# gsanya/orbslam2_NMI

Hardware: AMD Instinct MI355X
Metric: pose-candidate NMI evals/sec (640x480, 256 bins), one blocking nmi_search_grid call per step incl. its 8-byte read-back (SURVEY.md 8d's definition); beside the W warm-up steps an untimed clock warm-up of clock_warmup_ms = 200 ms precedes the timed region (higher is better)
Workload: dtype u8

## Files before the change

### orbslam2_nmi_amd/csrc/nmi_capi.cpp

```cpp
#include <sched.h>

#include "nmi_ctx.h"

namespace nmi_internal {

int hip_fail(nmi_ctx *ctx, hipError_t e, const char *what)
{
    if (ctx) {
        char buf[256];
        snprintf(buf, sizeof buf, "%s: %s (%d)", what, hipGetErrorString(e), (int)e);
        ctx->detail = buf;
    }
    return NMI_ERR_HIP - (int)e;
}



void build_order(int S, int Wn, int *order)
{
    const int tile_s = S >= 8 ? 8 : (S >= 4 ? 4 : (S >= 2 ? 2 : 1)), tile_w = 32 / tile_s;
    int64_t o = 0;
    for (int w0 = 0; w0 < Wn; w0 += tile_w)
        for (int s0 = 0; s0 < S; s0 += tile_s)
            for (int w = w0; w < w0 + tile_w && w < Wn; ++w)
                for (int s = s0; s < s0 + tile_s && s < S; ++s) order[o++] = w * S + s;
}

int ensure_order(nmi_ctx *ctx, int S, int Wn, const int **d_order)
{
    *d_order = nullptr;
    if (!ctx->xcd_tiling) return NMI_OK;
    const int64_t total = (int64_t)S * Wn;
    nmi_ctx::OrderEntry *victim = nullptr;
    for (auto &e : ctx->orders) {
        if (e.S == S && e.Wn == Wn) {
            e.last_use = ++ctx->order_clock;
            *d_order = e.d.as<int>();
            return NMI_OK;
        }
        if (!victim || (!e.d && victim->d) || (!e.d == !victim->d && e.last_use < victim->last_use)) victim = &e;
    }
    nmi_ctx::OrderEntry &e = *victim;
    if (e.d) NMI_HIP_TRY(ctx, hipStreamSynchronize(ctx->stream));
    e.S = e.Wn = -1;
    const size_t bytes = (size_t)total * sizeof(int);
    NMI_HIP_TRY(ctx, e.d.grow(bytes));
    NMI_HIP_TRY(ctx, e.h.grow(bytes, nmi_mem::kPinned));
    build_order(S, Wn, e.h.as<int>());
    NMI_HIP_TRY(ctx, hipMemcpyAsync(e.d.as<int>(), e.h.as<int>(), bytes, hipMemcpyHostToDevice, ctx->stream));
    e.S = S;
    e.Wn = Wn;
    e.last_use = ++ctx->order_clock;
    *d_order = e.d.as<int>();
    return NMI_OK;
}

nmi::PlanInputs plan_inputs(const nmi_ctx *ctx, nmi::SearchForm form, int64_t total, const nmi::GridArgs &a)
{
    nmi::PlanInputs in;
    in.compute_units = ctx->compute_units;
    in.workgroups = ctx->workgroups;
    in.hist_variant = ctx->hist_variant;
    in.split_mode = ctx->split_mode;
    in.split_pixels = ctx->split_pixels;
    in.shift = ctx->shift;
    in.use_bg = ctx->params.use_bg != 0;
    in.phase_mask = ctx->phase_mask;
    in.content_path = ctx->content_path;
    in.xcd_tiling = ctx->xcd_tiling != 0;
    in.cooldown = ctx->split_cooldown > 0;
    in.few_hint = ctx->few_hint;
    in.total = total;
    in.width = a.width;
    in.npix = ctx->npix;
    in.vec_ok = a.vec_ok != 0;
    in.form = form;
    return in;
}

double pix_owner_share(const nmi_ctx *ctx, int pix)
{
    const double owner_px = ((double)ctx->npix + (double)(pix - 1) * ctx->pix_owner_bias) / pix;
    return owner_px < ctx->npix ? owner_px / ctx->npix : 1.0;
}

static int ensure_pix_timeouts(nmi_ctx *ctx)
{
    NMI_HIP_TRY(ctx, ctx->d_pix_timeouts.grow(nmi::kPixHealWords * sizeof(uint32_t), ctx->stream, true));
    return NMI_OK;
}

static int next_split_epoch(nmi_ctx *ctx, uint32_t *epoch)
{
    uint32_t e = ctx->split_epoch + 1;
    if ((e & 0xFFFFu) == 0) {
        if (ctx->d_blocks) NMI_HIP_TRY(ctx, hipMemsetAsync(ctx->d_blocks.as<>(), 0, ctx->d_blocks.size(), ctx->stream));
        if (ctx->d_pix_blocks) NMI_HIP_TRY(ctx, hipMemsetAsync(ctx->d_pix_blocks.as<>(), 0, ctx->d_pix_blocks.size(), ctx->stream));
        if (e == 0 && ctx->d_slabs) NMI_HIP_TRY(ctx, hipMemsetAsync(ctx->d_slabs.as<>(), 0, ctx->d_slabs.size(), ctx->stream));
        ++e;
    }
    ctx->split_epoch = *epoch = e;
    return NMI_OK;
}

int prepare_pix_handoff(nmi_ctx *ctx, uint32_t *epoch)
{
    if (*epoch == 0) {
        const int rc = next_split_epoch(ctx, epoch);
        if (rc != NMI_OK) return rc;
    }
    return ensure_pix_timeouts(ctx);
}

static int ensure_zeroed(nmi_ctx *ctx, DeviceBuffer &buf, size_t bytes)
{
    NMI_HIP_TRY(ctx, buf.grow(bytes, ctx->stream, true));
    return NMI_OK;
}

int prepare_search(nmi_ctx *ctx, const nmi::SearchPlan &plan, nmi::GridArgs &a)
{
    const int64_t total = (int64_t)a.S_local * a.Wn;
    int rc = NMI_OK;
    if (plan.kind == nmi::SearchKernel::split) {
        rc = ensure_zeroed(ctx, ctx->d_slabs, (size_t)(total > 128 ? total : 128) * sizeof(nmi::SplitSlab));
        if (rc == NMI_OK && plan.pix_parts > 1) rc = ensure_zeroed(ctx, ctx->d_blocks, (size_t)total * nmi::split_block_bytes_per_candidate(plan.pix_parts));
        if (rc == NMI_OK) rc = next_split_epoch(ctx, &a.epoch);
        a.slabs = ctx->d_slabs.as<nmi::SplitSlab>();
        a.blocks = ctx->d_blocks.as<unsigned long long>();
        a.split_error = ctx->split_error.device<uint32_t>();
    } else if (plan.kind == nmi::SearchKernel::pix) {
        rc = ensure_zeroed(ctx, ctx->d_pix_blocks, nmi::pix_block_bytes((int)total, plan.pix));
        if (rc == NMI_OK) rc = prepare_pix_handoff(ctx, &a.epoch);
        a.blocks = ctx->d_pix_blocks.as<unsigned long long>();
    } else if (plan.order_table) {
        rc = ensure_order(ctx, a.S_local, a.Wn, &a.order);
    }
    if (rc != NMI_OK) return rc;
#ifdef NMI_BUILD_ABLATIONS
    if (plan.scratch && plan.workgroups > ctx->scratch_workgroups) {
        ctx->scratch_workgroups = 0;
        const int alloc = plan.workgroups > ctx->compute_units ? plan.workgroups : ctx->compute_units;
        NMI_HIP_TRY(ctx, ctx->d_scratch.grow(nmi::grid_kernel_scratch_bytes(alloc), ctx->stream));
        ctx->scratch_workgroups = alloc;
        a.scratch = ctx->d_scratch.as<uint32_t>();
    }
#endif
    if (plan.probe) a.plan = ctx->d_plan.as<nmi::LevelPlan>();
    if (plan.kind == nmi::SearchKernel::few_levels) {
        const size_t need = (size_t)(a.S_local + a.Wn) * (size_t)ctx->npix;
        if (need > ctx->d_rank_stacks.size()) NMI_HIP_TRY(ctx, ctx->d_rank_stacks.grow(need + need / 2, ctx->stream));
    }
    return NMI_OK;
}

int commit_launch(nmi_ctx *ctx, bool post, bool post_score, const SearchLaunch &rec, bool launched, SearchLaunch *out)
{
    if (post) ++ctx->seq;
    if (post_score) ++ctx->pair_seq;
    ctx->posted = post;
    ctx->last_slot = ctx->slot;
    ctx->last = rec;
    if (out) *out = rec;
    if (!launched) return NMI_OK;
    ctx->slot ^= 1;
    if (ctx->profiling) {
        NMI_HIP_TRY(ctx, hipEventRecord(ctx->ev_stop, ctx->stream));
        ctx->have_timing = true;
    }
    return NMI_OK;
}

nmi::GridArgs grid_args(const nmi_ctx *ctx, const SearchRequest &rq, bool post, bool post_score)
{
    const nmi_params &p = ctx->params;
    nmi::GridArgs a{};
    a.render_stack = rq.render_stack;
    a.warp_stack = rq.warp_stack;
    a.S_local = rq.S_local;
    a.Wn = rq.Wn;
    a.s_offset = rq.s_offset;
    a.S_total = rq.S_total;
    a.w_offset = rq.w_offset;
    nmi::set_geometry(a, p.width, p.height, rq.render_stack, rq.warp_stack, p.render_bottom_up != 0);
    a.shift = ctx->shift;
    a.mode = p.mode;
    a.ratings = rq.d_ratings;
    a.key = ctx->d_keys.as<unsigned long long>() + ctx->slot;
    a.reset_key = ctx->d_keys.as<unsigned long long>() + (ctx->slot ^ 1);
    a.out_key = rq.out_key;
    a.done = ctx->d_done.as<unsigned int>();
    a.mailbox = post ? ctx->mailbox.as<nmi::Mailbox>() : nullptr;
    a.score_post = post_score ? ctx->score_mailbox.as<unsigned long long>() : nullptr;
    a.seq = post ? ctx->seq + 1 : (post_score ? ctx->pair_seq + 1 : 0);
    a.hist_variant = ctx->hist_variant;
    return a;
}

int enqueue_grid(nmi_ctx *ctx, const SearchRequest &rq, SearchLaunch *launched)
{
    const nmi_params &p = ctx->params;
    const bool post = rq.post && ctx->result_path == 1, post_score = rq.post_score && ctx->result_path == 1;
    nmi::GridArgs a = grid_args(ctx, rq, post, post_score);
    if (rq.pair_renders) {
        a.pair_renders = rq.pair_renders;
        a.pair_warps = rq.pair_warps;
        uintptr_t bits = 0;
        for (int i = 0; i < rq.S_local; ++i) bits |= (uintptr_t)rq.pair_renders_host[i] | (uintptr_t)rq.pair_warps_host[i];
        if (bits % 16) nmi::set_geometry(a, p.width, p.height, (const void *)1, (const void *)1, p.render_bottom_up != 0);
    }
    a.table = ctx->table.as<float>();
    a.scratch = ctx->d_scratch.as<uint32_t>();
    a.dbg_joint = rq.dbg_joint;
    a.dbg_h1 = rq.dbg_h1;
    a.dbg_h2 = rq.dbg_h2;
    a.dbg_sums = rq.dbg_sums;
    a.dbg_stamps = ctx->dbg_stamps;

    const int64_t total = (int64_t)rq.S_local * rq.Wn;
// ... 673 lines not shown
```

### orbslam2_nmi_amd/csrc/nmi_ctx.h

```cpp
#pragma once
#include <hip/hip_runtime.h>
#include <math.h>
#include <stdio.h>
#include <string.h>

#include <new>
#include <string>
#include <vector>

#include "nmi_hip.h"
#include "nmi_covered.h"
#include "nmi_kernels.h"
#include "nmi_masked.h"
#include "nmi_mem.h"
#include "nmi_search_plan.h"
#include "nmi_tone.h"

struct SearchLaunch {
    nmi::SearchKernel kind = nmi::SearchKernel::none;
    int parts = 0;
    int pix = 0;
    uint32_t epoch = 0;
    int few = 0;
};

using nmi_mem::DeviceBuffer;
using nmi_mem::PinnedBuffer;

struct MeshWorkArea {
    DeviceBuffer zbuf, bins, state, clip_queue, clip_state, pairs, pair_state;
    nmi::MeshWork view;
};

struct nmi_ctx {
    nmi_params params{};
    int device = 0;
    int compute_units = 0;
    int npix = 0;
    int shift = 0;
    nmi_mem::Stream own_stream;
    hipStream_t stream = nullptr;
    DeviceBuffer table;
    DeviceBuffer d_keys;
    PinnedBuffer h_key;
    DeviceBuffer d_done;
    PinnedBuffer mailbox;
    unsigned int seq = 0;
    int slot = 0;
    int last_slot = 0;
    SearchLaunch last;
    int pix_owner_bias = 49152;
    DeviceBuffer d_pix_timeouts;
    uint32_t split_timeouts = 0;
    uint32_t split_cooldown = 0;
    uint32_t split_backoff = kSplitBackoffMin;
    uint32_t split_cooldown_epoch = 0;
    static constexpr uint32_t kSplitBackoffMin = 16, kSplitBackoffMax = 4096;
    int result_path = 1;
    bool posted = false;
    DeviceBuffer d_pair_rating;
    DeviceBuffer d_reduced_key;
    PinnedBuffer score_mailbox;
    unsigned int pair_seq = 0;
    int wait_mode = 0;
    struct OrderEntry {
        int S = -1, Wn = -1;
        DeviceBuffer d;
        PinnedBuffer h;
        uint64_t last_use = 0;
    };
    static constexpr int kOrderCache = 16;
    OrderEntry orders[kOrderCache];
    uint64_t order_clock = 0;
    int xcd_tiling = 1;
    DeviceBuffer d_slabs;
    DeviceBuffer d_blocks;
    uint32_t split_epoch = 0;
    PinnedBuffer split_error;
    DeviceBuffer d_pix_blocks;
    PinnedBuffer pair_table;
    DeviceBuffer d_pair_scores;
    int pairs_cap = 0;
    int split_pixels = -1;
    DeviceBuffer d_plan;
    PinnedBuffer level_post;
    uint32_t level_seq = 0;
    uint32_t level_seen = 0;
    bool few_hint = false;
    int content_path = -1;
    int fewlevels_bins = 4096;
    DeviceBuffer d_rank_stacks;
    unsigned long long *dbg_stamps = nullptr;
    int stamp_candidate = 0;
    int split_mode = -1;
    DeviceBuffer d_zbuf;
    DeviceBuffer d_no_red;
    MeshWorkArea mesh;
    int mesh_views = 0;
    unsigned long long tile_queue_limit = 4ull << 20;
    unsigned long long clip_queue_limit = ~0ull;
    nmi_mem::UploadRing mvp_ring, warp_ring;
    DeviceBuffer d_scratch;
    int scratch_workgroups = 0;
    DeviceBuffer d_mask_counts;
    DeviceBuffer d_mask_tables;
    int mask_count_n = 0;
    DeviceBuffer d_mask_redo;
    DeviceBuffer d_mask_redo_state;
    DeviceBuffer d_cover_counts;
    int64_t cover_count_n = 0;
    nmi::ToneSetting tone;
    nmi_internal::ToneWork tone_work;
    nmi::ValidRange valid;
    nmi_mem::Event ev_start, ev_stop;
    int hist_variant = 3;
    int phase_mask = 3;
    int workgroups = 0;
    bool profiling = false;
    bool have_timing = false;
    std::string detail;
};

struct nmi_texture {
    nmi_ctx *ctx = nullptr;
    DeviceBuffer d_luma;
    int levels = 0;
    int w[16] = {}, h[16] = {};
    long long off[16] = {};
};

namespace nmi_internal {

int mesh_work_alloc(nmi_ctx *ctx, int S, MeshWorkArea *w);
int ensure_mesh_work(nmi_ctx *ctx, int S);
int ensure_mesh_pairs(nmi_ctx *ctx, MeshWorkArea *w, long long n_triangles);
int warp_inverse_coeffs(const double *forward , float *coeffs );
int point_sprite_size(float point_size, int *size);
int level_enqueue(nmi_level *lv, const float *h_mvps, const double *h_forward, const unsigned long long **d_key);
nmi_ctx *level_ctx(nmi_level *lv);
int rccl_allreduce_key(nmi_ctx *ctx, const unsigned long long *d_send, unsigned long long *d_recv, void *nccl_comm);

int hip_fail(nmi_ctx *ctx, hipError_t e, const char *what);
void build_order(int S, int Wn, int *order);
int ensure_order(nmi_ctx *ctx, int S, int Wn, const int **d_order);
struct SearchRequest {
    const uint8_t *render_stack = nullptr, *warp_stack = nullptr;
    int S_local = 0, s_offset = 0, S_total = 0, Wn = 0, w_offset = 0;
    float *d_ratings = nullptr;
    unsigned long long *out_key = nullptr;
    bool post = false;
    bool post_score = false;
    uint32_t *dbg_joint = nullptr, *dbg_h1 = nullptr, *dbg_h2 = nullptr;
    float *dbg_sums = nullptr;
    bool caller_checks_split = false;
    const uint8_t *const *pair_renders = nullptr, *const *pair_warps = nullptr;
    const uint8_t *const *pair_renders_host = nullptr, *const *pair_warps_host = nullptr;
    static SearchRequest block(const uint8_t *renders, int S_local, int s_offset, int S_total, const uint8_t *warps, int Wn, int w_offset = 0)
    {
        SearchRequest rq;
        rq.render_stack = renders;
        rq.warp_stack = warps;
        rq.S_local = S_local;
        rq.s_offset = s_offset;
        rq.S_total = S_total;
        rq.Wn = Wn;
        rq.w_offset = w_offset;
        return rq;
    }
};
struct MaskSide {
    const uint8_t *warp_masks = nullptr, *render_masks = nullptr;
    int32_t *counts = nullptr;
    const float *tables = nullptr;
    int32_t *redo = nullptr;
    uint32_t *redo_state = nullptr;
};
nmi::GridArgs grid_args(const nmi_ctx *ctx, const SearchRequest &rq, bool post, bool post_score);
nmi::PlanInputs plan_inputs(const nmi_ctx *ctx, nmi::SearchForm form, int64_t total, const nmi::GridArgs &a);
double pix_owner_share(const nmi_ctx *ctx, int pix);
int prepare_pix_handoff(nmi_ctx *ctx, uint32_t *epoch);
int prepare_search(nmi_ctx *ctx, const nmi::SearchPlan &plan, nmi::GridArgs &a);
int commit_launch(nmi_ctx *ctx, bool post, bool post_score, const SearchLaunch &rec, bool launched, SearchLaunch *out);
int enqueue_grid(nmi_ctx *ctx, const SearchRequest &rq, SearchLaunch *launched = nullptr);
struct MaskSearch {
    bool covered;
    nmi::MaskedGridArgs masked;
    nmi::CoveredGridArgs cover;
};
MaskSearch mask_search_args(const nmi::GridArgs &a, const MaskSide &m);
hipError_t launch_mask_search(const MaskSearch &ms, int pix, double owner_share, int workgroups, bool use_bg, bool exact,
                              const uint32_t *replay, uint32_t *healed, hipStream_t stream);
int ensure_mask_redo(nmi_ctx *ctx, int64_t total);
int enqueue_grid_mask(nmi_ctx *ctx, const SearchRequest &rq, const MaskSide &m, SearchLaunch *launched = nullptr);
int wait_word(nmi_ctx *ctx, const volatile unsigned long long *word, unsigned long long mask, unsigned long long want,
              unsigned long long *out);
int stage_floats(nmi_ctx *ctx, nmi_mem::UploadRing &ring, const float *h_src, size_t n, float **d_out);
int fetch_key(nmi_ctx *ctx, unsigned long long *key);
bool split_timed_out(nmi_ctx *ctx);
bool split_launch_failed(nmi_ctx *ctx, const SearchLaunch &launch);
extern const char *const kSplitTimeoutNote, *const kSplitTimeoutTicketNote, *const kSplitTimeoutTicketLost;
int search_block(nmi_ctx *ctx, const uint8_t *render_stack, int32_t S_local, int32_t s_offset, int32_t S_total, const uint8_t *warp_stack,
                 int32_t Wn_local, int32_t w_offset, int32_t Wn_total, float *d_ratings, uint64_t *d_key, uint64_t *h_key,
                 bool caller_checks);
enum class MapKind { points, textured_mesh, colored_mesh };
int render_points_impl(nmi_ctx *ctx, const float *d_xyz, const float *d_red, int64_t n_points, const float *h_mvps, int32_t S,
                       float point_size, uint8_t *d_render_stack, uint8_t *cover, const nmi::DepthShade *depth = nullptr);
int render_mesh_impl(nmi_ctx *ctx, MapKind kind, const float *d_xyz, const float *d_attr, int64_t n_triangles, const nmi_texture *tex,
                     const float *h_mvps, int32_t S, uint8_t *d_render_stack, uint8_t *cover, const nmi::DepthShade *depth = nullptr);
int depth_shade_check(const nmi_depth_shade *shade, nmi::DepthShade *out);
nmi::MeshShading mesh_shading(MapKind kind, const float *d_attr, const nmi_texture *tex);
nmi::RenderTarget render_target(const nmi_ctx *ctx, uint8_t *out, uint8_t *cover, const nmi::DepthShade *depth);
nmi::MeshLimits mesh_limits(const nmi_ctx *ctx, int layout_views);
int check_grid_args(nmi_ctx *ctx, const uint8_t *render_stack, int S_local, int s_offset, int S_total, const uint8_t *warp_stack,
                    int Wn);

#define NMI_HIP_TRY(ctx, call)                                  \
    do {                                                        \
        hipError_t e_ = (call);                                 \
        if (e_ != hipSuccess) return nmi_internal::hip_fail((ctx), e_, #call); \
    } while (0)

struct FirstError {
    hipError_t e = hipSuccess;
    bool operator()(hipError_t r)
    {
        if (e == hipSuccess) e = r;
        return r == hipSuccess;
// ... 18 lines not shown
```

### orbslam2_nmi_amd/csrc/nmi_grid_device.h

```cpp
#pragma once
#include <hip/hip_runtime.h>
#include <stdint.h>

#include "nmi_kernels.h"
#include "nmi_device.h"

namespace nmi {

namespace {

constexpr int kBlock = NMI_BLOCK_THREADS;
constexpr int kWaves = kBlock / 64;
constexpr int kBins = 256;
constexpr int kWords = kBins * kBins / 2;
constexpr int kRowStride = 129;
constexpr int kJointWords = kBins * kRowStride;
constexpr int kOvfCap = 1024;
constexpr int kRowsPerWave = kBins / kWaves;
constexpr int kLdsTable = 4096;
constexpr int kSide = 8;


struct Lds {
    uint32_t joint[kJointWords];
// ... 260 lines not shown
                const int cn = min(ch + kStep, last);
                const uint4 wn = ldw(cn), rn = ldr(cn);
                add_chunk<BG, SHIFTED, HIST, true>(lds, par, rc, wc, a.shift, try_flat);
                wc = wn;
                rc = rn;
            }
        }
        if (ROWS && row_rem > 0) {
            const int x0 = a.chunks_per_row << 4, n = a.height * row_rem;
            for (int t = tid; t < n; t += NT) {
                const int y = t / row_rem, x = x0 + t - y * row_rem;
                const int ry = a.flip ? (a.height - 1 - y) : y;
                uint32_t d1 = render[ry * a.width + x], d2 = warped[y * a.width + x];
                if (HIST == 2) {
                    if (BG || (d1 != 0 && d2 != 0)) {
                        if (SHIFTED) {
                            d1 >>= a.shift;
                            d2 >>= a.shift;
                        }
                        (void)__hip_atomic_fetch_add(&lds.joint[joint_word(d1, d2)], joint_inc(d2), __ATOMIC_RELAXED, __HIP_MEMORY_SCOPE_WORKGROUP);
                    }
                } else {
                    add_pixel<BG, SHIFTED>(lds, par, d1, d2, a.shift);
                }
            }
        }
    } else {
        for (int pos = tid; pos < a.npix; pos += NT) {
            const int y = pos / a.width;
            const int x = pos - y * a.width;
            const int ry = a.flip ? (a.height - 1 - y) : y;
            if (HIST == 2) {
                uint32_t d1 = render[ry * a.width + x], d2 = warped[pos];
                if (BG || (d1 != 0 && d2 != 0)) {
                    if (SHIFTED) {
                        d1 >>= a.shift;
                        d2 >>= a.shift;
                    }
                    (void)__hip_atomic_fetch_add(&lds.joint[joint_word(d1, d2)], joint_inc(d2), __ATOMIC_RELAXED,
                                                 __HIP_MEMORY_SCOPE_WORKGROUP);
                }
            } else {
                add_pixel<BG, SHIFTED>(lds, par, render[ry * a.width + x], warped[pos], a.shift);
            }
        }
    }
}

__device__ __forceinline__ float term(const float *__restrict__ table, uint32_t c)
{
    return c ? table[c] : 0.0f;
}
__device__ __forceinline__ float term_lds(const Lds &lds, const float *__restrict__ table, uint32_t c)
{
    float t = lds.table[c < (uint32_t)kLdsTable ? c : 0u];
    if (__builtin_expect(c >= (uint32_t)kLdsTable, 0)) t = table[c];
    return t;
}

static_assert(kWaves == 16 && (kWaves * kRowStride) % 32 == 16, "rows kWaves apart must fall on opposite halves of the 32 banks");
__device__ __forceinline__ int decode_row(int wave, int pass, int r) { return wave + 4 * kWaves * pass + kWaves * r; }
__device__ __forceinline__ bool in_decode_pass(uint32_t d1, int wave, int pass)
{
    return (d1 % (uint32_t)kWaves) == (uint32_t)wave && (d1 / (uint32_t)(4 * kWaves)) == (uint32_t)pass;
}
__device__ __forceinline__ uint32_t decode_word(int d1, int i, int k) { return (uint32_t)(d1 * kRowStride + i + 16 * k); }

__device__ __forceinline__ void apply_wraps(const Lds &lds, int par, uint32_t novf, uint32_t word, uint32_t &lo,
                                            uint32_t &hi)
{
    for (uint32_t e = 0; e < novf; ++e) {
        const uint32_t ev = lds.ovf[par][e];
        if ((ev >> 1) == word) {
            if (ev & 1u) {
                hi += 65536u;
            } else {
                lo += 65536u;
                hi -= 1u;
            }
        }
    }
}

template <bool ZERO0 = false>
__device__ __forceinline__ void decode_phase(Lds &lds, int par, const GridArgs &a, int wave, int lane)
{
    const uint32_t novf = lds.ovf_n[par] < (uint32_t)kOvfCap ? lds.ovf_n[par] : (uint32_t)kOvfCap;
    const bool side_any = lds.side_key[par][0] != 0u;
    uint32_t wave_total = 0;
    const int i = lane & 15, r = lane >> 4;
    uint32_t col_lo[8], col_hi[8];
#pragma unroll
    for (int k = 0; k < 8; ++k) col_lo[k] = col_hi[k] = 0;
#pragma unroll 1
    for (int pass = 0; pass < kRowsPerWave / 4; ++pass) {
        const int d1 = decode_row(wave, pass, r);
        const uint32_t a0 = decode_word(d1, i, 0);
        uint32_t lo[8], hi[8];
#pragma unroll
        for (int k = 0; k < 8; ++k) {
            const uint32_t idx = a0 + 16 * k;
            const uint32_t wd = lds.joint[idx];
            lds.joint[idx] = 0;
            lo[k] = wd & 0xFFFFu;
            hi[k] = wd >> 16;
        }
        if (__builtin_expect(novf != 0, 0)) {
#pragma unroll
            for (int k = 0; k < 8; ++k) apply_wraps(lds, par, novf, a0 + 16 * k, lo[k], hi[k]);
        }
        if (__builtin_expect(side_any, 0)) {
            for (int e = 0; e < kSide; ++e) {
                const uint32_t key1 = __builtin_amdgcn_readfirstlane(lds.side_key[par][e]);
                if (key1 == 0u) break;
                const uint32_t sd1 = (key1 - 1u) >> 8, sd2 = (key1 - 1u) & 0xFFu;
                if (!in_decode_pass(sd1, wave, pass)) continue;
                const uint32_t sword = joint_word(sd1, sd2);
                const uint32_t cnt = lds.side_cnt[par][e];
#pragma unroll
                for (int k = 0; k < 8; ++k) {
                    if (a0 + 16 * k == sword) {
                        if (sd2 & 128u)
                            hi[k] += cnt;
                        else
                            lo[k] += cnt;
                    }
                }
            }
        }
        uint32_t rsum = 0, cmax = 0;
        if (ZERO0) {
            uint32_t raw = 0;
#pragma unroll
            for (int k = 0; k < 8; ++k) raw += lo[k] + hi[k];
            wave_total += row_sum_16(raw);
            if (i == 0) lo[0] = 0;
            if (d1 == 0) {
#pragma unroll
                for (int k = 0; k < 8; ++k) lo[k] = hi[k] = 0;
            }
        }
        float tl[8], th[8];
#pragma unroll
        for (int k = 0; k < 8; ++k) {
            col_lo[k] += lo[k];
            col_hi[k] += hi[k];
            rsum += lo[k] + hi[k];
            cmax = max(cmax, max(lo[k], hi[k]));
            tl[k] = lds.table[lo[k] & (kLdsTable - 1)];
            th[k] = lds.table[hi[k] & (kLdsTable - 1)];
        }
        if (__builtin_expect(cmax >= (uint32_t)kLdsTable, 0)) {
#pragma unroll
            for (int k = 0; k < 8; ++k) {
                if (lo[k] >= (uint32_t)kLdsTable) tl[k] = a.table[lo[k]];
                if (hi[k] >= (uint32_t)kLdsTable) th[k] = a.table[hi[k]];
            }
        }
        rsum = row_sum_16(rsum);
        if (!ZERO0) wave_total += rsum;
        const float x = row_tree_16(lane_tree_16(tl, th));
        if (i == 0) {
            lds.hist_render[d1] = rsum;
            lds.joint_row_sums[d1] = x;
        }
        if (a.dbg_joint) {
            uint32_t *row = a.dbg_joint + d1 * kBins;
#pragma unroll
            for (int k = 0; k < 8; ++k) {
                const int q = i + 16 * k;
                row[q] = lo[k];
                row[q + 128] = hi[k];
            }
        }
    }
#pragma unroll
    for (int k = 0; k < 8; ++k) {
        const int q = i + 16 * k;
        atomicAdd(&lds.hist_warped[q], col_lo[k]);
        atomicAdd(&lds.hist_warped[q + 128], col_hi[k]);
    }
    if (i == 0) atomicAdd(&lds.total[par], wave_total);
}

__device__ __forceinline__ void final_phase(Lds &lds, const GridArgs &a, int lane, int p, int w, int s,
                                            unsigned long long &prev_key)
{
    const int i = lane & 15, r = lane >> 4;
    float lo[8], hi[8];
    const uint32_t *h = r == 0 ? lds.hist_render : lds.hist_warped;
    uint32_t cl[8], ch[8];
#pragma unroll
    for (int k = 0; k < 8; ++k) {
        cl[k] = r < 2 ? h[i + 16 * k] : 0u;
        ch[k] = r < 2 ? h[i + 16 * k + 128] : 0u;
    }
#pragma unroll
    for (int k = 0; k < 8; ++k) {
        lo[k] = a.table[cl[k]];
        hi[k] = a.table[ch[k]];
    }
    if ((w == 0 || s == 0) && a.plan) {
        uint32_t m = 0;
#pragma unroll
        for (int k = 0; k < 8; ++k) m |= (cl[k] != 0u ? 1u << k : 0u) | (ch[k] != 0u ? 0x100u << k : 0u);
        if (lane < 32 && m) __hip_atomic_fetch_or(const_cast<uint32_t *>(&a.plan->seen[lane]), m, __ATOMIC_RELAXED, __HIP_MEMORY_SCOPE_AGENT);
    }
    if (r == 2) {
#pragma unroll
        for (int k = 0; k < 8; ++k) {
            lo[k] = lds.joint_row_sums[i + 16 * k];
            hi[k] = lds.joint_row_sums[i + 16 * k + 128];
        }
    }
    const float x = row_tree_16(lane_tree_16(lo, hi));
    const float a1 = __shfl(x, 0, 64), a2 = __shfl(x, 16, 64), a3 = __shfl(x, 32, 64);
    if (a.dbg_h1 && lane < 64) {
        for (int t = lane; t < kBins; t += 64) {
            a.dbg_h1[t] = lds.hist_render[t];
            if (a.dbg_h2) a.dbg_h2[t] = lds.hist_warped[t];
        }
    }
    if (lane == 0) commit_score(a, p, w, s, a1, a2, a3, prev_key);
}

__device__ __forceinline__ void finish_search(const GridArgs &a, int lane, unsigned long long prev_key, uint32_t expected)
{
    LevelPlan *plan = const_cast<LevelPlan *>(a.plan);
    uint32_t arrived = 0;
    if (lane == 0) {
        const unsigned int one = prev_key == ~0ull ? 2u : 1u;
        arrived = __hip_atomic_fetch_add(a.done, one, __ATOMIC_RELAXED, __HIP_MEMORY_SCOPE_AGENT);
    }
    if (__builtin_amdgcn_readfirstlane(arrived) != expected - 1) return;
    unsigned long long final_key = 0;
    uint32_t bits = 0;
    unsigned long long *post = nullptr;
    uint32_t state = 0, max_joint = 0;
    if (lane == 0) final_key = __hip_atomic_load(a.key, __ATOMIC_RELAXED, __HIP_MEMORY_SCOPE_AGENT);
    if (plan && lane < 32) bits = __hip_atomic_exchange(&plan->seen[lane], 0u, __ATOMIC_RELAXED, __HIP_MEMORY_SCOPE_AGENT);
    if (plan && lane == 0) post = plan->seen_post, state = plan->seen_state, max_joint = plan->seen_max_joint;
    if (lane == 0) {
        __hip_atomic_store(a.done, 0u, __ATOMIC_RELAXED, __HIP_MEMORY_SCOPE_AGENT);
        if (a.out_key) __hip_atomic_store(a.out_key, final_key, __ATOMIC_RELAXED, __HIP_MEMORY_SCOPE_SYSTEM);
        if (a.mailbox)
            __hip_atomic_store(&a.mailbox->word, final_key | ((unsigned long long)(a.seq & 1u) << 63), __ATOMIC_RELAXED, __HIP_MEMORY_SCOPE_SYSTEM);
    }
    if (plan) {
        const uint32_t n = row_sum_16((uint32_t)__popc(bits));
        const uint32_t nw = (uint32_t)__shfl((int)n, 16, 64);
        const uint32_t few = (n > 0u && nw > 0u && n * nw <= max_joint) ? 1u : 0u;
        if (lane == 0 && post && few != state) {
            plan->seen_state = few;
            const uint32_t stamp = 0x80000000u | (uint32_t)wall_clock64();
            __hip_atomic_store(post, ((unsigned long long)stamp << 32) | ((unsigned long long)n << 16) | nw, __ATOMIC_RELAXED, __HIP_MEMORY_SCOPE_SYSTEM);
        }
    }
}

template <bool SHIFTED, bool BG = true, bool ROWS = false>
__device__ __forceinline__ void exact_candidate(Lds &lds, const GridArgs &a, int tid, int p, unsigned long long &prev_key)
{
    const int lane = tid & 63, wave = tid >> 6;
    const int w = p / a.S_local, s = p - w * a.S_local;
    __syncthreads();
    histogram_phase<true, SHIFTED, 1, kBlock, true, ROWS>(lds, 0, a, a.render_stack + (size_t)s * a.npix, a.warp_stack + (size_t)w * a.npix, tid, 0,
                                                          ROWS ? a.height * a.chunks_per_row : a.npix >> 4);
    __syncthreads();
    decode_phase<!BG>(lds, 0, a, wave, lane);
    __syncthreads();
    if (wave == 0) {
        final_phase(lds, a, lane, p, w, s, prev_key);
        for (int t = lane; t < kBins; t += 64) lds.hist_warped[t] = 0;
        if (lane == 0) lds.ovf_n[0] = lds.total[0] = 0;
        if (lane < kSide) lds.side_key[0][lane] = lds.side_cnt[0][lane] = 0;
    }
    __syncthreads();
}

}

}
```

### orbslam2_nmi_amd/csrc/nmi_kernels.hip

```cpp
#include <hip/hip_runtime.h>
#include <stdint.h>

#include "nmi_grid_device.h"

namespace nmi {

#if defined(NMI_GRID_KERNEL_GATED)
#define NMI_GRID_KERNEL_NAME nmi_grid_kernel_gated
#elif defined(NMI_GRID_KERNEL_STAMPED)
#define NMI_GRID_KERNEL_NAME nmi_grid_kernel_stamped
#elif defined(NMI_GRID_KERNEL_ROWS)
#define NMI_GRID_KERNEL_NAME nmi_grid_kernel_rows
#else
#define NMI_GRID_KERNEL_NAME nmi_grid_kernel
#endif
#ifdef NMI_GRID_KERNEL_STAMPED
#define NMI_GRID_STAMP(k)                                                                                         \
    do {                                                                                                          \
        if (a.dbg_stamps && tid == ((k) == 7 ? 64 : 0) && stamp_on) a.dbg_stamps[blockIdx.x * 8 + (k)] = wall_clock64(); \
    } while (0)
#else
#define NMI_GRID_STAMP(k) \
    do {                  \
    } while (0)
#endif
#ifndef NMI_WAVE_SLABS
#define NMI_WAVE_SLABS 1
#endif
#ifdef NMI_GRID_KERNEL_STAMPED
namespace {
__device__ uint32_t stamp_candidate = 0;
}
#endif
template <bool BG, bool SHIFTED, int HIST>
__global__ __launch_bounds__(NMI_BLOCK_THREADS) void NMI_GRID_KERNEL_NAME(GridArgs a)
{
    __shared__ Lds lds;
#ifdef NMI_GRID_KERNEL_GATED
    if (a.plan->use != 0u) return;
#endif
    const int tid = threadIdx.x;
    const int lane = tid & 63;
    const int wave = tid >> 6;
#ifdef NMI_GRID_KERNEL_STAMPED
    bool stamp_on = true;
    const int stamp_ordinal = slot_in_round(blockIdx.x, gridDim.x) + (int)stamp_candidate * (int)gridDim.x;
#endif
    NMI_GRID_STAMP(0);
    constexpr bool kOptimistic = HIST == 3;
    constexpr int kFirst = kOptimistic ? 2 : HIST;
#ifdef NMI_GRID_KERNEL_ROWS
    constexpr bool kRows = true;
#define NMI_ALL_CHUNKS (a.height * a.chunks_per_row)
#else
    constexpr bool kRows = false;
#define NMI_ALL_CHUNKS (a.npix >> 4)
#endif
    constexpr bool kZero0 = !BG && kOptimistic && !SHIFTED;
    constexpr bool kCountAll = BG || kZero0;
    constexpr bool kSlabs = NMI_WAVE_SLABS != 0 && kFirst == 2;

    if (blockIdx.x == 0 && tid == 0 && a.reset_key) *a.reset_key = 0ull;
    float tab[kLdsTable / kBlock];
#pragma unroll
    for (int k = 0; k < kLdsTable / kBlock; ++k) {
        const int c = tid + k * kBlock;
        tab[k] = a.table[c <= a.npix ? c : 0];
    }
    {
        uint4 *j4 = reinterpret_cast<uint4 *>(lds.joint);
        const uint4 z = {0, 0, 0, 0};
        for (int i = tid; i < kJointWords / 4; i += kBlock) j4[i] = z;
    }
    if (tid < kBins) lds.hist_warped[tid] = 0;
    if (tid < 2) lds.ovf_n[tid] = lds.total[tid] = 0;
    if (tid < 2 * kSide) (&lds.side_key[0][0])[tid] = (&lds.side_cnt[0][0])[tid] = 0;
    bool table_pending = true;
    int exact_from = -1;
    __syncthreads();
    NMI_GRID_STAMP(1);

    const int total = a.S_local * a.Wn;
    unsigned long long prev_key = 0;
    int par = 0;
    const int slot = slot_in_round(blockIdx.x, gridDim.x);
    int ordinal = slot;
    for (; ordinal < total; ordinal += gridDim.x, par ^= 1) {
        const int p = candidate_at(a, ordinal);
        const int w = p / a.S_local;
        const int s = p - w * a.S_local;
        const uint8_t *render = a.render_stack + (size_t)s * a.npix;
        const uint8_t *warped = a.warp_stack + (size_t)w * a.npix;
#ifdef NMI_GRID_KERNEL_STAMPED
        stamp_on = ordinal == stamp_ordinal;
#endif
        NMI_GRID_STAMP(7);

        if (a.phase_mask & 1) {
            if (a.phase_mask & 8) {
                if (wave < kWaves / 2) histogram_phase<kCountAll, SHIFTED, kFirst, kBlock / 2, true, kRows>(lds, par, a, render, warped, tid, 0, NMI_ALL_CHUNKS);
            } else
                histogram_phase<kCountAll, SHIFTED, kFirst, kBlock, true, kRows, kSlabs>(lds, par, a, render, warped, tid, 0, NMI_ALL_CHUNKS, ordinal != slot);
        }
        if (table_pending) {
#pragma unroll
            for (int k = 0; k < kLdsTable / kBlock; ++k) lds.table[tid + k * kBlock] = tab[k];
            table_pending = false;
        }
        NMI_GRID_STAMP(2);
#ifdef NMI_GRID_KERNEL_STAMPED
        if (a.dbg_stamps && lane == 0 && stamp_on) a.dbg_stamps[gridDim.x * 8 + blockIdx.x * 16 + wave] = wall_clock64();
#endif
        __syncthreads();
        NMI_GRID_STAMP(3);
        if (a.phase_mask & 2) decode_phase<kZero0>(lds, par, a, wave, lane);
        __syncthreads();
        NMI_GRID_STAMP(4);
        if (kOptimistic && (a.phase_mask & 3) == 3 && lds.total[par] != (uint32_t)a.npix) {
            exact_from = ordinal;
            break;
        }
        if (wave == 0) {
            if (a.phase_mask & 2) final_phase(lds, a, lane, p, w, s, prev_key);
            for (int t = lane; t < kBins; t += 64) lds.hist_warped[t] = 0;
            if (lane == 0) {
                lds.ovf_n[par] = 0;
                lds.total[par ^ 1] = 0;
            }
            if (lane < kSide) {
                int l = lane;
                asm volatile("" : "+v"(l));
                lds.side_key[par][l] = lds.side_cnt[par][l] = 0;
            }
        }
        NMI_GRID_STAMP(5);
    }

    if (kOptimistic && exact_from >= 0) {
        __syncthreads();
        if (tid < kBins) lds.hist_warped[tid] = 0;
        if (tid < 2) lds.total[tid] = lds.ovf_n[tid] = 0;
        if (tid < 2 * kSide) (&lds.side_key[0][0])[tid] = (&lds.side_cnt[0][0])[tid] = 0;
        __syncthreads();
        for (int o = exact_from; o < total; o += gridDim.x) exact_candidate<SHIFTED, !kZero0, kRows>(lds, a, tid, candidate_at(a, o), prev_key);
    }

    if (wave == 0 && !(a.phase_mask & 16)) {
        finish_search(a, lane, prev_key, gridDim.x);
    }
#ifdef NMI_GRID_KERNEL_STAMPED
    stamp_on = true;
#endif
    NMI_GRID_STAMP(6);
}

#if defined(NMI_GRID_KERNEL_ROWS)
hipError_t launch_grid_rows(const GridArgs &a, int workgroups, bool use_bg, hipStream_t stream)
{
    if (a.width < 32 || (a.hist_variant != 1 && a.hist_variant != 3)) return hipErrorInvalidValue;
    const dim3 grid(workgroups), block(kBlock);
    const bool exact_only = a.hist_variant == 1 || (!use_bg && a.shift != 0);
    if (exact_only) {
        if (use_bg) {
            if (a.shift != 0) hipLaunchKernelGGL((nmi_grid_kernel_rows<true, true, 1>), grid, block, 0, stream, a);
            else hipLaunchKernelGGL((nmi_grid_kernel_rows<true, false, 1>), grid, block, 0, stream, a);
        } else {
            if (a.shift != 0) hipLaunchKernelGGL((nmi_grid_kernel_rows<false, true, 1>), grid, block, 0, stream, a);
            else hipLaunchKernelGGL((nmi_grid_kernel_rows<false, false, 1>), grid, block, 0, stream, a);
        }
    } else if (a.shift != 0) {
        hipLaunchKernelGGL((nmi_grid_kernel_rows<true, true, 3>), grid, block, 0, stream, a);
    } else if (use_bg) {
        hipLaunchKernelGGL((nmi_grid_kernel_rows<true, false, 3>), grid, block, 0, stream, a);
    } else {
        hipLaunchKernelGGL((nmi_grid_kernel_rows<false, false, 3>), grid, block, 0, stream, a);
    }
    return hipGetLastError();
}
#elif defined(NMI_GRID_KERNEL_STAMPED)
hipError_t set_stamped_experiment(int k, const uint32_t *cum)
{
    const uint32_t kk = (uint32_t)k;
    hipError_t e = hipMemcpyToSymbol(HIP_SYMBOL(stamp_candidate), &kk, sizeof kk);
    if (e == hipSuccess && cum) {
        for (int r = 0; r < 2; ++r)
            for (int v = 0; v <= kWaves; ++v) {
                const uint32_t c = cum[r * (kWaves + 1) + v];
                if (c > 65536u || (v == 0 && c != 0u) || (v == kWaves && c != 65536u) || (v > 0 && c < cum[r * (kWaves + 1) + v - 1])) return hipErrorInvalidValue;
            }
        e = hipMemcpyToSymbol(HIP_SYMBOL(slab_cum), cum, 2 * (kWaves + 1) * sizeof(uint32_t));
    }
    return e;
}

hipError_t launch_grid_stamped(const GridArgs &a, int workgroups, hipStream_t stream)
{
    if (a.hist_variant != 3 || a.shift != 0) return hipErrorInvalidValue;
    hipLaunchKernelGGL((nmi_grid_kernel_stamped<true, false, 3>), dim3(workgroups), dim3(kBlock), 0, stream, a);
    return hipGetLastError();
}
#elif defined(NMI_GRID_KERNEL_GATED)
hipError_t launch_grid_gated(const GridArgs &a, int workgroups, bool use_bg, hipStream_t stream)
{
    if (a.hist_variant != 3 || !a.plan || (a.shift != 0 && !use_bg)) return hipErrorInvalidValue;
    const dim3 grid(workgroups), block(kBlock);
    if (a.shift != 0)
        hipLaunchKernelGGL((nmi_grid_kernel_gated<true, true, 3>), grid, block, 0, stream, a);
// ... 285 lines not shown
```

### orbslam2_nmi_amd/csrc/nmi_search_plan.h

```cpp
#pragma once
#include <stdint.h>

#if defined(__HIPCC__)
#define NMI_PLAN_HD __host__ __device__
#else
#define NMI_PLAN_HD
#endif

namespace nmi {

NMI_PLAN_HD inline bool split_exact_grid(int total, int parts) { return total < 8 && parts == 8; }
NMI_PLAN_HD inline int split_workgroups(int candidates, int parts, int pix_parts)
{
    return (split_exact_grid(candidates, parts) ? candidates : ((candidates + 7) / 8) * 8) * parts * pix_parts;
}
constexpr int kPixMaxRanges = 5;

enum class SearchForm { plain, masked, level };
enum class SearchKernel { none, grid, split, pix, few_levels };

struct PlanInputs {
    int compute_units = 0;
    int workgroups = 0;
    int hist_variant = 3;
    int split_mode = -1;
    int split_pixels = -1;
    int shift = 0;
    bool use_bg = true;
    int phase_mask = 3;
    int content_path = -1;
    bool xcd_tiling = true;
    bool cooldown = false;
    bool few_hint = false;
    int64_t total = 0;
    int width = 0, npix = 0;
    bool vec_ok = false;
    bool debug_exports = false, stamps = false, pair_pointers = false;
    bool split_checked = false;
    SearchForm form = SearchForm::plain;
};

struct SearchPlan {
    SearchKernel kind = SearchKernel::none;
    int parts = 0;
    int pix_parts = 1;
    int pix = 0;
    int workgroups = 0;
    int phase_mask = 3;
    bool order_table = false;
    bool probe = false;
    bool scratch = false;
    bool used_cooldown = false;
    bool read_hint = false;
    bool unsupported = false;
};

inline int plan_cap(int workgroups_option, int compute_units) { return workgroups_option > 0 ? workgroups_option : compute_units; }
inline int grid_workgroups(int64_t total, int workgroups_option, int compute_units)
{
    const int cap = plan_cap(workgroups_option, compute_units);
    return (int)(total < cap ? total : cap);
}

inline void plan_split(const PlanInputs &in, int cap, int *parts, int *pix_parts)
{
    *parts = 0;
    *pix_parts = 1;
    const int64_t total = in.total;
    if (cap > in.compute_units) cap = in.compute_units;
    if (in.hist_variant != 3 || in.split_mode == 0 || in.split_mode == 1 || total <= 0 || total > cap) return;
    auto fits = [&](int k, int p) { return split_workgroups((int)total, k, p) <= cap; };
    auto exists = [](int k, int p) { return p == 1 || (k == 8 && (p == 2 || p == 4)) || (k == 4 && p == 2); };
    const int want_p = in.split_pixels;
    if (in.split_mode > 0) {
        const int k = in.split_mode;
        if (!fits(k, 1)) return;
        *parts = k;
        if (want_p == 1) return;
        for (int p = 4; p >= 2; p >>= 1)
            if ((want_p == -1 || want_p == p) && exists(k, p) && fits(k, p)) {
                *pix_parts = p;
                return;
            }
        return;
    }
    static const int order[][2] = {{8, 4}, {8, 2}, {4, 2}, {8, 1}, {4, 1}};
    for (const auto &kp : order) {
        if (kp[1] > 1 && want_p != -1 && want_p != kp[1]) continue;
        if (fits(kp[0], kp[1])) {
            *parts = kp[0];
            *pix_parts = kp[1];
            return;
        }
    }
}

inline int plan_pix(const PlanInputs &in, int cap)
{
    const int64_t total = in.total;
    const bool stamps = in.stamps && in.form == SearchForm::plain;
    if (cap > in.compute_units) cap = in.compute_units;
    if (in.hist_variant != 3 || in.width < 32 || (in.shift != 0 && !in.use_bg) || in.pair_pointers || total <= 0) return 0;
    if ((in.phase_mask & ~512) != 3 || (stamps && in.split_mode != 1)) return 0;
    if (in.split_mode == 1) {
        const int p = in.split_pixels;
        return (p >= 2 && p <= kPixMaxRanges && total * p <= cap) ? p : 0;
    }
    if (in.split_mode != -1 || in.split_pixels != -1 || total * 2 > cap) return 0;
    const int p = (int)(cap / total);
    if (!in.vec_ok) return p > kPixMaxRanges ? kPixMaxRanges : p;
    if (total <= 32) return 0;
    return p > 3 ? 3 : p;
}

inline SearchPlan plan_search(const PlanInputs &in)
{
    SearchPlan plan;
    if (in.total <= 0) return plan;
    const int cap = plan_cap(in.workgroups, in.compute_units);
    plan.workgroups = grid_workgroups(in.total, in.workgroups, in.compute_units);
    plan.pix = plan_pix(in, cap);
    if (in.form != SearchForm::plain) {
        plan.kind = plan.pix ? SearchKernel::pix : SearchKernel::grid;
        plan.phase_mask = plan.pix ? 3 | (in.phase_mask & 512) : 3;
        plan.order_table = !plan.pix && (in.form == SearchForm::level || (in.xcd_tiling && in.total <= (1ll << 24)));
        return plan;
    }
    plan.phase_mask = in.phase_mask;
    plan_split(in, cap, &plan.parts, &plan.pix_parts);
    if (plan.pix_parts > 1 && in.npix >= (1 << 24)) plan.pix_parts = 1;
    if (plan.pix) plan.parts = 0;
    if (plan.parts && !in.split_checked) plan.parts = 0;
    if (plan.parts && in.cooldown) {
        plan.used_cooldown = true;
        plan.parts = 0;
    }
    if (!plan.parts) plan.pix_parts = 1;
    plan.read_hint = !plan.parts && !(plan.pix && in.split_mode == 1) && in.vec_ok && (in.shift == 0 || in.use_bg) && in.hist_variant == 3 &&
                     in.phase_mask == 3 && !in.debug_exports && !in.pair_pointers && !in.stamps && in.content_path != 0;
    const bool few = plan.read_hint && (in.content_path == 1 || in.few_hint);
    if (few) plan.pix = 0;
    if (in.pair_pointers && !plan.parts) {
        plan.unsupported = true;
        plan.workgroups = 0;
        return plan;
    }
    if (plan.parts) {
        plan.kind = SearchKernel::split;
        plan.workgroups = split_workgroups((int)in.total, plan.parts, plan.pix_parts);
    } else if (plan.pix) {
        plan.kind = SearchKernel::pix;
        plan.workgroups = (int)in.total * plan.pix;
    } else {
        plan.kind = few ? SearchKernel::few_levels : SearchKernel::grid;
        plan.order_table = in.xcd_tiling && in.total <= (1ll << 24);
    }
    plan.scratch = in.hist_variant == 4;
    plan.probe = !plan.parts && in.hist_variant == 3 && in.content_path != 0;
    return plan;
}

}
```

Baseline: 9.134 million.

## Order candidates so workgroups reuse warped-image histogram across consecutive iterations

Adds a shared search order that assigns each workgroup a run of consecutive candidates sharing the same warp index. When the warp matches the previous iteration, the kernel skips re-accumulating the warped marginal histogram and its LDS clearing, and reuses the cached frame sum. The order table is now keyed on grid size as well. This only applies in the optimistic background-enabled variant and adds complexity in the host-side order construction, with a fallback to tile order when the divisibility constraints fail.

Measured after the change: 9.526 million, median of 6. +4.3%, better.

```diff
diff --git a/orbslam2_nmi_amd/csrc/nmi_capi.cpp b/orbslam2_nmi_amd/csrc/nmi_capi.cpp
--- a/orbslam2_nmi_amd/csrc/nmi_capi.cpp
+++ b/orbslam2_nmi_amd/csrc/nmi_capi.cpp
@@ -16,24 +16,16 @@
 
 
 
-void build_order(int S, int Wn, int *order)
-{
-    const int tile_s = S >= 8 ? 8 : (S >= 4 ? 4 : (S >= 2 ? 2 : 1)), tile_w = 32 / tile_s;
-    int64_t o = 0;
-    for (int w0 = 0; w0 < Wn; w0 += tile_w)
-        for (int s0 = 0; s0 < S; s0 += tile_s)
-            for (int w = w0; w < w0 + tile_w && w < Wn; ++w)
-                for (int s = s0; s < s0 + tile_s && s < S; ++s) order[o++] = w * S + s;
-}
-
-int ensure_order(nmi_ctx *ctx, int S, int Wn, const int **d_order)
+void build_order(int S, int Wn, int *order) { nmi::build_tile_order(S, Wn, order); }
+
+int ensure_order(nmi_ctx *ctx, int S, int Wn, int grid, const int **d_order)
 {
     *d_order = nullptr;
     if (!ctx->xcd_tiling) return NMI_OK;
     const int64_t total = (int64_t)S * Wn;
     nmi_ctx::OrderEntry *victim = nullptr;
     for (auto &e : ctx->orders) {
-        if (e.S == S && e.Wn == Wn) {
+        if (e.S == S && e.Wn == Wn && e.grid == grid) {
             e.last_use = ++ctx->order_clock;
             *d_order = e.d.as<int>();
             return NMI_OK;
@@ -46,10 +38,12 @@
     const size_t bytes = (size_t)total * sizeof(int);
     NMI_HIP_TRY(ctx, e.d.grow(bytes));
     NMI_HIP_TRY(ctx, e.h.grow(bytes, nmi_mem::kPinned));
-    build_order(S, Wn, e.h.as<int>());
+    if (grid > 0) nmi::build_search_order(S, Wn, grid, e.h.as<int>());
+    else build_order(S, Wn, e.h.as<int>());
     NMI_HIP_TRY(ctx, hipMemcpyAsync(e.d.as<int>(), e.h.as<int>(), bytes, hipMemcpyHostToDevice, ctx->stream));
     e.S = S;
     e.Wn = Wn;
+    e.grid = grid;
     e.last_use = ++ctx->order_clock;
     *d_order = e.d.as<int>();
     return NMI_OK;
@@ -134,7 +128,7 @@
         if (rc == NMI_OK) rc = prepare_pix_handoff(ctx, &a.epoch);
         a.blocks = ctx->d_pix_blocks.as<unsigned long long>();
     } else if (plan.order_table) {
-        rc = ensure_order(ctx, a.S_local, a.Wn, &a.order);
+        rc = ensure_order(ctx, a.S_local, a.Wn, plan.shared_order ? plan.workgroups : 0, &a.order);
     }
     if (rc != NMI_OK) return rc;
 #ifdef NMI_BUILD_ABLATIONS
diff --git a/orbslam2_nmi_amd/csrc/nmi_ctx.h b/orbslam2_nmi_amd/csrc/nmi_ctx.h
--- a/orbslam2_nmi_amd/csrc/nmi_ctx.h
+++ b/orbslam2_nmi_amd/csrc/nmi_ctx.h
@@ -65,6 +65,7 @@
     int wait_mode = 0;
     struct OrderEntry {
         int S = -1, Wn = -1;
+        int grid = 0;
         DeviceBuffer d;
         PinnedBuffer h;
         uint64_t last_use = 0;
@@ -142,7 +143,7 @@
 
 int hip_fail(nmi_ctx *ctx, hipError_t e, const char *what);
 void build_order(int S, int Wn, int *order);
-int ensure_order(nmi_ctx *ctx, int S, int Wn, const int **d_order);
+int ensure_order(nmi_ctx *ctx, int S, int Wn, int grid, const int **d_order);
 struct SearchRequest {
     const uint8_t *render_stack = nullptr, *warp_stack = nullptr;
     int S_local = 0, s_offset = 0, S_total = 0, Wn = 0, w_offset = 0;
diff --git a/orbslam2_nmi_amd/csrc/nmi_grid_device.h b/orbslam2_nmi_amd/csrc/nmi_grid_device.h
--- a/orbslam2_nmi_amd/csrc/nmi_grid_device.h
+++ b/orbslam2_nmi_amd/csrc/nmi_grid_device.h
@@ -366,7 +366,7 @@
     }
 }
 
-template <bool ZERO0 = false>
+template <bool ZERO0 = false, bool KEPT = false>
 __device__ __forceinline__ void decode_phase(Lds &lds, int par, const GridArgs &a, int wave, int lane)
 {
     const uint32_t novf = lds.ovf_n[par] < (uint32_t)kOvfCap ? lds.ovf_n[par] : (uint32_t)kOvfCap;
@@ -427,8 +427,10 @@
         float tl[8], th[8];
 #pragma unroll
         for (int k = 0; k < 8; ++k) {
-            col_lo[k] += lo[k];
-            col_hi[k] += hi[k];
+            if (!KEPT) {
+                col_lo[k] += lo[k];
+                col_hi[k] += hi[k];
+            }
             rsum += lo[k] + hi[k];
             cmax = max(cmax, max(lo[k], hi[k]));
             tl[k] = lds.table[lo[k] & (kLdsTable - 1)];
@@ -458,17 +460,19 @@
             }
         }
     }
-#pragma unroll
-    for (int k = 0; k < 8; ++k) {
-        const int q = i + 16 * k;
-        atomicAdd(&lds.hist_warped[q], col_lo[k]);
-        atomicAdd(&lds.hist_warped[q + 128], col_hi[k]);
+    if (!KEPT) {
+#pragma unroll
+        for (int k = 0; k < 8; ++k) {
+            const int q = i + 16 * k;
+            atomicAdd(&lds.hist_warped[q], col_lo[k]);
+            atomicAdd(&lds.hist_warped[q + 128], col_hi[k]);
+        }
     }
     if (i == 0) atomicAdd(&lds.total[par], wave_total);
 }
 
 __device__ __forceinline__ void final_phase(Lds &lds, const GridArgs &a, int lane, int p, int w, int s,
-                                            unsigned long long &prev_key)
+                                            unsigned long long &prev_key, bool kept = false, float *frame_sum = nullptr)
 {
     const int i = lane & 15, r = lane >> 4;
     float lo[8], hi[8];
@@ -476,8 +480,8 @@
     uint32_t cl[8], ch[8];
 #pragma unroll
     for (int k = 0; k < 8; ++k) {
-        cl[k] = r < 2 ? h[i + 16 * k] : 0u;
-        ch[k] = r < 2 ? h[i + 16 * k + 128] : 0u;
+        cl[k] = r < (kept ? 1 : 2) ? h[i + 16 * k] : 0u;
+        ch[k] = r < (kept ? 1 : 2) ? h[i + 16 * k + 128] : 0u;
     }
 #pragma unroll
     for (int k = 0; k < 8; ++k) {
@@ -498,7 +502,12 @@
         }
     }
     const float x = row_tree_16(lane_tree_16(lo, hi));
-    const float a1 = __shfl(x, 0, 64), a2 = __shfl(x, 16, 64), a3 = __shfl(x, 32, 64);
+    const float a1 = __shfl(x, 0, 64), a3 = __shfl(x, 32, 64);
+    float a2 = __shfl(x, 16, 64);
+    if (frame_sum) {
+        if (kept) a2 = *frame_sum;
+        else *frame_sum = __uint_as_float(__builtin_amdgcn_readfirstlane(__float_as_uint(a2)));
+    }
     if (a.dbg_h1 && lane < 64) {
         for (int t = lane; t < kBins; t += 64) {
             a.dbg_h1[t] = lds.hist_render[t];
diff --git a/orbslam2_nmi_amd/csrc/nmi_kernels.hip b/orbslam2_nmi_amd/csrc/nmi_kernels.hip
--- a/orbslam2_nmi_amd/csrc/nmi_kernels.hip
+++ b/orbslam2_nmi_amd/csrc/nmi_kernels.hip
@@ -59,6 +59,7 @@
     constexpr bool kZero0 = !BG && kOptimistic && !SHIFTED;
     constexpr bool kCountAll = BG || kZero0;
     constexpr bool kSlabs = NMI_WAVE_SLABS != 0 && kFirst == 2;
+    constexpr bool kKeepWarp = kOptimistic && BG;
 
     if (blockIdx.x == 0 && tid == 0 && a.reset_key) *a.reset_key = 0ull;
     float tab[kLdsTable / kBlock];
@@ -83,6 +84,9 @@
     const int total = a.S_local * a.Wn;
     unsigned long long prev_key = 0;
     int par = 0;
+    int kept_w = -1;
+    float frame_sum = 0.0f;
+    const bool keep_ok = kKeepWarp && !a.dbg_h1 && !a.dbg_h2;
     const int slot = slot_in_round(blockIdx.x, gridDim.x);
     int ordinal = slot;
     for (; ordinal < total; ordinal += gridDim.x, par ^= 1) {
@@ -113,7 +117,12 @@
 #endif
         __syncthreads();
         NMI_GRID_STAMP(3);
-        if (a.phase_mask & 2) decode_phase<kZero0>(lds, par, a, wave, lane);
+        const bool kept = keep_ok && w == kept_w && !(s == 0 && a.plan);
+        if (a.phase_mask & 2) {
+            if (kKeepWarp && kept) decode_phase<false, true>(lds, par, a, wave, lane);
+            else decode_phase<kZero0>(lds, par, a, wave, lane);
+        }
+        kept_w = w;
         __syncthreads();
         NMI_GRID_STAMP(4);
         if (kOptimistic && (a.phase_mask & 3) == 3 && lds.total[par] != (uint32_t)a.npix) {
@@ -121,8 +130,9 @@
             break;
         }
         if (wave == 0) {
-            if (a.phase_mask & 2) final_phase(lds, a, lane, p, w, s, prev_key);
-            for (int t = lane; t < kBins; t += 64) lds.hist_warped[t] = 0;
+            if (a.phase_mask & 2) final_phase(lds, a, lane, p, w, s, prev_key, kept, kKeepWarp ? &frame_sum : nullptr);
+            if (!kept)
+                for (int t = lane; t < kBins; t += 64) lds.hist_warped[t] = 0;
             if (lane == 0) {
                 lds.ovf_n[par] = 0;
                 lds.total[par ^ 1] = 0;
diff --git a/orbslam2_nmi_amd/csrc/nmi_search_plan.h b/orbslam2_nmi_amd/csrc/nmi_search_plan.h
--- a/orbslam2_nmi_amd/csrc/nmi_search_plan.h
+++ b/orbslam2_nmi_amd/csrc/nmi_search_plan.h
@@ -48,6 +48,7 @@
     int workgroups = 0;
     int phase_mask = 3;
     bool order_table = false;
+    bool shared_order = false;
     bool probe = false;
     bool scratch = false;
     bool used_cooldown = false;
@@ -154,10 +155,72 @@
     } else {
         plan.kind = few ? SearchKernel::few_levels : SearchKernel::grid;
         plan.order_table = in.xcd_tiling && in.total <= (1ll << 24);
+        plan.shared_order = plan.order_table && !few;
     }
     plan.scratch = in.hist_variant == 4;
     plan.probe = !plan.parts && in.hist_variant == 3 && in.content_path != 0;
     return plan;
 }
 
-}
+
+inline void build_tile_order(int S, int Wn, int *order)
+{
+    const int tile_s = S >= 8 ? 8 : (S >= 4 ? 4 : (S >= 2 ? 2 : 1)), tile_w = 32 / tile_s;
+    int64_t o = 0;
+    for (int w0 = 0; w0 < Wn; w0 += tile_w)
+        for (int s0 = 0; s0 < S; s0 += tile_s)
+            for (int w = w0; w < w0 + tile_w && w < Wn; ++w)
+                for (int s = s0; s < s0 + tile_s && s < S; ++s) order[o++] = w * S + s;
+}
+
+inline int order_slot_at(int pos, int grid)
+{
+    if ((grid & 7) == 0) return pos;
+    for (int x = 0; x < 8; ++x) {
+        const int n = (grid - x + 7) / 8;
+        if (pos < n) return x + 8 * pos;
+        pos -= n;
+    }
+    return -1;
+}
+
+inline bool build_shared_order(int S, int Wn, int grid, int *order)
+{
+    const int64_t total = (int64_t)S * Wn;
+    if (S < 2 || Wn < 2 || grid < 1 || total <= grid) return false;
+    const int R = (int)((total + grid - 1) / grid);
+    const int A = (int)(total - (int64_t)(R - 1) * grid);
+    const int B = grid - A;
+    const int y0 = (R - S % R) % R;
+    if ((int64_t)y0 * (R - 1) > S) return false;
+    const int x0 = (S - y0 * (R - 1)) / R;
+    const int64_t rest = (int64_t)B - (int64_t)Wn * y0;
+    if (rest < 0 || rest % R) return false;
+    const int64_t J = rest / R;
+    const int jmax = x0 / (R - 1);
+    if (J > (int64_t)Wn * jmax) return false;
+    const int j_all = (int)(J / Wn), j_more = (int)(J % Wn);
+    for (int kind = 0; kind < 2; ++kind) {
+        int pos = 0;
+        for (int v = 0; v < Wn; ++v) {
+            const int w = kind == 0 ? v : Wn - 1 - v;
+            const int j = j_all + (w >= Wn - j_more ? 1 : 0);
+            const int x = x0 - j * (R - 1), y = y0 + j * R, m = x + y;
+            for (int t = kind == 0 ? 0 : x; t < (kind == 0 ? x : m); ++t) {
+                int slot;
+                do slot = order_slot_at(pos++, grid);
+                while ((slot < A) != (kind == 0));
+                const int n = kind == 0 ? R : R - 1;
+                for (int k = 0; k < n; ++k) order[slot + (int64_t)k * grid] = w * S + k * m + t;
+            }
+        }
+    }
+    return true;
+}
+
+inline void build_search_order(int S, int Wn, int grid, int *order)
+{
+    if (!build_shared_order(S, Wn, grid, order)) build_tile_order(S, Wn, order);
+}
+
+}
```
